# tvlearn/evo

Hardware: AMD Instinct MI355X
Metric: E-step candidate-state evals/sec (NxS), full EM iteration (higher is better)
Workload: dtype f64; 1 GPU; ES3C D=256 H=512 S=200 N=100k f64 (north-star shape); algo=es3c, N_total=100000, N_rank0=100000, D=256, H=512, S=200, step=10 full EM iterations, world_size_rccl=1, ea=fit/randflip 10 parents x 1 child x 1 gen, states=p_init_Kn=1/H (init_states default), rng=device, mstep=device, parallelism=dp1

## Files before the change

evo_amd/csrc/evo_amd.hip:

```cpp
#include "../../include/evo_amd.h"

#include <dlfcn.h>
#include <math.h>
#include <stdarg.h>
#include <stdio.h>
#include <stdlib.h>
#include <string.h>

#include <chrono>
#include <memory>
#include <string>
#include <vector>

#include "common.hpp"
#include "gemm_f64.hpp"
#include "kernels_bsc.hpp"
#include "kernels_common.hpp"
#include "kernels_evolve.hpp"
#include "kernels_mstep.hpp"
#include "kernels_sssc.hpp"
#include "kernels_sssc_quad.hpp"
#include "kernels_fused.hpp"

static thread_local char g_err[512] = "";
// ... 110 lines not shown
  bool gemm_forked = false;
  hipStream_t stream_copy = nullptr;
  hipEvent_t ev_theta = nullptr, ev_theta_done = nullptr;
  hipEvent_t ev_mbox = nullptr, ev_bak = nullptr;
  int mbox_side = 1;
  int theta_copy_engine = 0;
  double rel_frac = -1.0;
  bool ar_gemm_pending = false;
  int overlap_gemm = 1;
  int early_fork = -1;
  int bg_unit = 0;
  int fold_clear = 1;
  bool acc_clean = false, clist_clean = false;
  bool wq_copy_valid = false;
  double *gram_diag_out = nullptr;
  bool gram_diag_written = false;
  bool mbox_fold_req = false;
  unsigned long long mbox_folded_seq = 0;
  int stats_chunks = 1;
  int n_cu = 256;
  int stats_stage = 1;
  int stats_waves = 0;
  PairBins pbins = {};
  int bins_min = 256;
 int bins_scale = 3;
  int bins_scale_cur = 0;
  int bins_auto = 1;
  int bins_nwg = 2048;
  int bsc_wave_opt = 1;
  int gemm_ws_opt = 1;
  double *gemm_ws = nullptr;
  size_t gemm_ws_n = 0;
  int pair_bins = 1;
  int gemm_streamk = 1;
  int fork_spare = 0;
  int sk_spare = -1;
  int sssc_prec32 = 0;
  int main_unstaged = 1;
  int sing_screen = 1;
  double *huge = nullptr;
  int *huge_ctl = nullptr;
  int huge_slots = 0, huge_kc = 0;
  int *sing_gen = nullptr;
  int theta_gen = 0;
  int gemm_grouped = 1;
  int gemm_per_xcd = 0;
  double grid_scale = 1.0;
  double *census = nullptr;
  i64 pre_n = 4;
  hipEvent_t ev_chunk[16] = {};
  bool configured = false, have_data = false, have_params = false, have_cand = false, B_valid = false;
  bool need_known = false;
  bool res_need[3] = {true, true, true};
  double res_cnt[3] = {0, 0, 0};
  bool cand_from_device = false;
  bool lists_clean = false;
  int pending_skip = 0;
  bool conservative_levels = false;
  int pays_agreed = -1;
  int k8_mode = -1;
  bool bsc_direct = false;
  bool f32_opt = false, f32 = false;
  float *Yf = nullptr, *Ytf = nullptr, *Wf = nullptr, *Bf = nullptr, *Esf = nullptr;
  i64 ldYt = 0;
  double *Yt = nullptr;
  int b_tn_opt = 1;
// ... 221 lines not shown
  HIP_TRY(hipEventCreateWithFlags(&c->ev_theta, hipEventDisableTiming));
  HIP_TRY(hipEventCreateWithFlags(&c->ev_theta_done, hipEventDisableTiming));
  HIP_TRY(hipEventCreateWithFlags(&c->ev_mbox, hipEventDisableTiming));
  HIP_TRY(hipEventCreateWithFlags(&c->ev_bak, hipEventDisableTiming));
  for (int i = 0; i < 16; i++) HIP_TRY(hipEventCreateWithFlags(&c->ev_chunk[i], hipEventDisableTiming));

  HIP_TRY(hipFuncSetAttribute((const void *)sssc_stats_flat_kernel, hipFuncAttributeMaxDynamicSharedMemorySize, 150 * 1024));
  HIP_TRY(hipFuncSetAttribute((const void *)sssc_big_kernel<0>, hipFuncAttributeMaxDynamicSharedMemorySize,
                              136 * 1024));
  HIP_TRY(hipFuncSetAttribute((const void *)sssc_big_kernel<0, 0>, hipFuncAttributeMaxDynamicSharedMemorySize,
                              136 * 1024));
  HIP_TRY(hipFuncSetAttribute((const void *)sssc_big_kernel<0, 1>, hipFuncAttributeMaxDynamicSharedMemorySize,
                              136 * 1024));
  HIP_TRY(hipFuncSetAttribute((const void *)sssc_big_kernel<1>, hipFuncAttributeMaxDynamicSharedMemorySize,
                              136 * 1024));
  HIP_TRY(hipFuncSetAttribute((const void *)gemm_tn128_f64, hipFuncAttributeMaxDynamicSharedMemorySize,
                              (int)GEMM128_LDS_BYTES));
  HIP_TRY(hipFuncSetAttribute((const void *)gemm_tn128_rows_f64, hipFuncAttributeMaxDynamicSharedMemorySize,
                              (int)GEMM128_LDS_BYTES));
  HIP_TRY(hipFuncSetAttribute((const void *)gemm_tn128_sk_f64, hipFuncAttributeMaxDynamicSharedMemorySize,
                              (int)GEMM128_LDS_BYTES));
  HIP_TRY(hipFuncSetAttribute((const void *)gemm_tn128_sk_f32, hipFuncAttributeMaxDynamicSharedMemorySize,
                              (int)GEMM128_LDS_BYTES));
  HIP_TRY(hipFuncSetAttribute((const void *)gemm_tn128_store_f32, hipFuncAttributeMaxDynamicSharedMemorySize,
                              (int)GEMM128_LDS_BYTES));
  {
    const void *wk[] = {(const void *)sssc_stats_wave_kernel<0, 4>,  (const void *)sssc_stats_wave_kernel<1, 4>,
                        (const void *)sssc_stats_wave_kernel<2, 4>,  (const void *)sssc_stats_wave_kernel<4, 4>,
                        (const void *)sssc_stats_wave_kernel<8, 4>,  (const void *)sssc_stats_wave_kernel<16, 4>,
                        (const void *)sssc_stats_wave_kernel<0, 1>,  (const void *)sssc_stats_wave_kernel<0, 8>,
                        (const void *)sssc_stats_wave_kernel<0, 16>};
    for (const void *f : wk) HIP_TRY(hipFuncSetAttribute(f, hipFuncAttributeMaxDynamicSharedMemorySize, 150 * 1024));
    HIP_TRY(hipFuncSetAttribute((const void *)pair_bins_reduce_kernel, hipFuncAttributeMaxDynamicSharedMemorySize, 3 * PB_TILE * 8));
    HIP_TRY(hipFuncSetAttribute((const void *)sssc_small_kernel<4, 1, 2, 256>, hipFuncAttributeMaxDynamicSharedMemorySize, 120 * 1024));
    HIP_TRY(hipFuncSetAttribute((const void *)sssc_small_kernel<8, 1, 2, 256>, hipFuncAttributeMaxDynamicSharedMemorySize, 120 * 1024));
  }
  {
    const void *fk[] = {(const void *)sssc_estep_fused_kernel<1, false>,  (const void *)sssc_estep_fused_kernel<1, true>,
                        (const void *)sssc_estep_fused_kernel<2, false>,  (const void *)sssc_estep_fused_kernel<2, true>,
                        (const void *)sssc_estep_fused_kernel<4, false>,  (const void *)sssc_estep_fused_kernel<4, true>,
                        (const void *)sssc_estep_fused_kernel<8, false>,  (const void *)sssc_estep_fused_kernel<8, true>,
                        (const void *)sssc_estep_fused_kernel<16, false>, (const void *)sssc_estep_fused_kernel<16, true>};
    for (const void *fp : fk) HIP_TRY(hipFuncSetAttribute(fp, hipFuncAttributeMaxDynamicSharedMemorySize, 160 * 1024));
  }
  *out = c;
  return 0;
}

static void free_all(evoamd_ctx *c) {
  void *ptrs[] = {c->Y,      c->yy,     c->y2sum,   c->states,  c->cand,     c->lpj,       c->cand_lpj,
                  c->cand_counts, c->flags, c->rowmax, c->rowsum, c->partial, c->partial2, c->diag, c->stage,    c->W,
                  c->Wt,     c->G,      c->Psi,     c->Bm,      c->mus,      c->pilbar_v,  c->GP,      c->DG,    c->D1,    c->PT,   c->yhat,  c->tmpWt,  c->mask_infr,  c->mask_x,  c->Yrec,
                  c->pies,   c->tmpA,    c->tmpB,    c->tmpC,    c->gjwork,  c->colpart,
                  c->acc_base, c->Es,     c->list1,   c->list2,    c->list3,    c->list_n,    c->err,
                  c->tmp_y,  c->tmp_lpj, c->tmp_states, c->dig, c->cand_dig, c->lpj_alt, c->cand_raw, c->dupold, c->gen_start,
                  c->pbins.ent, c->pbins.part, c->pbins.gcnt, c->gemm_ws, c->Yt, c->Yf, c->Ytf, c->Wf, c->Bf, c->Esf,
                  c->clist, c->clist_n, c->ovf_rec, c->theta_bak, c->rowF, c->rowcnt, c->defer, c->fpart, c->huge, c->huge_ctl};
  for (void *p : ptrs)
    if (p) (void)hipFree(p);
  if (c->h_acc) (void)hipHostFree(c->h_acc);
  if (c->h_par) (void)hipHostFree(c->h_par);
  if (c->h_theta) (void)hipHostFree(c->h_theta);
  c->h_theta = nullptr;
  if (c->h_err) (void)hipHostFree(c->h_err);
  if (c->h_dpar) (void)hipHostFree(c->h_dpar);
}

extern "C" void evoamd_ctx_destroy(evoamd_ctx *c) {
  if (!c) return;
  (void)hipSetDevice(c->device);
  (void)hipStreamSynchronize(c->stream);
  if (c->comm && g_rccl.CommDestroy) g_rccl.CommDestroy(c->comm);
  for (auto &s : c->spans) {
    (void)hipEventDestroy(s.a);
    (void)hipEventDestroy(s.b);
  }
  for (auto e : c->pool) (void)hipEventDestroy(e);
  free_all(c);
  (void)hipStreamDestroy(c->stream);
  if (c->stream2) (void)hipStreamDestroy(c->stream2);
  if (c->stream_copy) (void)hipStreamDestroy(c->stream_copy);
  if (c->ev_theta) (void)hipEventDestroy(c->ev_theta);
  if (c->ev_theta_done) (void)hipEventDestroy(c->ev_theta_done);
  if (c->ev_mbox) (void)hipEventDestroy(c->ev_mbox);
  if (c->ev_bak) (void)hipEventDestroy(c->ev_bak);
  if (c->ev_fork) (void)hipEventDestroy(c->ev_fork);
  if (c->ev_join) (void)hipEventDestroy(c->ev_join);
  for (int i = 0; i < 16; i++)
    if (c->ev_chunk[i]) (void)hipEventDestroy(c->ev_chunk[i]);
// ... 14 lines not shown
  }
  if (strcmp(name, "bsc_direct") == 0) {
    c->bsc_direct = value != 0;
    c->have_params = false;
    return 0;
  }
  if (strcmp(name, "reconstruct_in_stats") == 0) {
    c->rec_in_stats = value != 0;
    return 0;
  }
  if (strcmp(name, "prefetch_lpj") == 0) {
    c->prefetch_lpj = value != 0;
    return 0;
  }
  if (strcmp(name, "inverse_block") == 0) {
    if (value != 0 && value != 16 && value != 32) return fail(EVOAMD_E_INVALID, "inverse_block: 0 (auto), 16 or 32");
    c->spd_block = value;
    return 0;
  }
  if (strcmp(name, "overlap_gemm") == 0) {
    c->overlap_gemm = value;
    return 0;
  }
  if (strcmp(name, "stats_stage") == 0) {
    c->stats_stage = value;
    return 0;
  }
  if (strcmp(name, "stats_waves") == 0) {
    c->stats_waves = value;
    return 0;
  }
  if (strcmp(name, "pair_bins") == 0) {
    c->pair_bins = value;
    return 0;
  }
  if (strcmp(name, "gemm_streamk") == 0) {
    c->gemm_streamk = value;
    return 0;
  }
  if (strcmp(name, "b_transposed") == 0) {
    c->b_tn_opt = value;
    return 0;
  }
  if (strcmp(name, "pair_bins_scale") == 0) {
    if (value < 1 || value > 64) return fail(EVOAMD_E_INVALID, "pair_bins_scale: 1 .. 64");
    c->bins_scale = value;
    return 0;
  }
  if (strcmp(name, "pair_bins_nwg") == 0) {
    if (value < 256 || value > 2048 || (value % 256) != 0) return fail(EVOAMD_E_INVALID, "pair_bins_nwg: 256 .. 2048, multiple of 256");
    c->bins_nwg = value;
    return 0;
  }
  if (strcmp(name, "pair_bins_auto") == 0) {
    c->bins_auto = value != 0;
    return 0;
  }
  if (strcmp(name, "pair_bins_min") == 0) {
    c->bins_min = value;
    return 0;
  }
  if (strcmp(name, "bsc_stats_wave") == 0) {
    c->bsc_wave_opt = value;
    return 0;
  }
  if (strcmp(name, "gemm_workspace") == 0) {
// ... 99 lines not shown
  return (c->model == EVOAMD_MODEL_BSC) ? H * D + H * H + H + 1 + 8 : 2 * H + 4 * H * H + D * H + D + 8;
}
struct AccLayout {
  i64 Wp, Wq, pies, sigma;
  i64 xs, xss, xsz, xszsz, s_sz, sz_sz, sWp, y2;
  i64 tail;
};
static AccLayout acc_layout(const evoamd_ctx *c) {
  AccLayout a = {};
  const i64 H = c->H, D = c->D;
  if (c->model == EVOAMD_MODEL_BSC) {
    a.Wp = 0;
    a.Wq = H * D;
    a.pies = a.Wq + H * H;
    a.sigma = a.pies + H;
    a.tail = a.sigma + 1;
  } else {
    a.xs = 0;
    a.xss = H;
    a.xsz = a.xss + H * H;
    a.xszsz = a.xsz + H;
    a.sWp = a.xszsz + H * H;
    a.s_sz = a.sWp + D * H;
    a.sz_sz = a.s_sz + H * H;
    a.y2 = a.sz_sz + H * H;
    a.tail = a.y2 + D;
  }
  return a;
}

static int alloc_pair_bins(evoamd_ctx *c, int scale) {
  const i64 N = c->N;
  const int H = c->H, S = c->S;
  if (c->pbins.ent) (void)hipFree(c->pbins.ent);
  if (c->pbins.gcnt) (void)hipFree(c->pbins.gcnt);
  if (c->pbins.part) (void)hipFree(c->pbins.part);
  c->pbins = PairBins{};
  c->bins_scale_cur = 0;
  if (H >= 2 && H <= 1024) {
    PairBins pb = {};
    pb.rf = std::max(1, PB_TILE / (2 * H));
    const int nfold = (H - 1 + 1) / 2;
    pb.nb = (int)cdiv(nfold, pb.rf);
    pb.nwg = c->bins_nwg;
    pb.nsh = std::max((i64)N * S >= (i64)8 << 20 ? 8 : 4, std::min(PB_NSH_MAX, 256 / std::max(1, pb.nb)));
    pb.cap = (int)std::max<i64>(64, (i64)scale * cdiv((i64)N * S, (i64)pb.nb * pb.nwg));
    const size_t ne = (size_t)pb.nb * pb.nwg * pb.cap;
    const bool got = hipMalloc((void **)&pb.ent, ne * sizeof(double4)) == hipSuccess &&
                     hipMalloc((void **)&pb.part, (size_t)pb.nb * pb.nsh * 3 * 2 * pb.rf * H * sizeof(double)) == hipSuccess &&
                     hipMalloc((void **)&pb.gcnt, (size_t)pb.nb * pb.nwg * sizeof(int)) == hipSuccess;
    if (got) {
      HIP_TRY(hipMemsetAsync(pb.gcnt, 0, (size_t)pb.nb * pb.nwg * sizeof(int), c->stream));
      c->pbins = pb;
      c->bins_scale_cur = scale;
    } else {
      (void)hipGetLastError();
      if (pb.ent) (void)hipFree(pb.ent);
      if (pb.part) (void)hipFree(pb.part);
      if (pb.gcnt) (void)hipFree(pb.gcnt);
    }
  }
  return 0;
}

static int ensure_bins_capacity(evoamd_ctx *c) {
  if (c->model != EVOAMD_MODEL_SSSC || !c->need_known || !c->pbins.ent || c->bins_auto == 0) return 0;
  const double NS = (double)c->N * c->S;
  const double n34 = c->res_cnt[0] - c->res_cnt[1], n58 = c->res_cnt[1] - c->res_cnt[2];
  const double entries = (NS - c->res_cnt[0]) + 6.0 * n34 + 28.0 * n58;
  int want = (int)std::ceil(3.0 * 1.25 * entries / NS);
  if (want > 64) want = 64;
  if (want <= c->bins_scale_cur) return 0;
  HIP_TRY(hipStreamSynchronize(c->stream));
  if (c->stream2) HIP_TRY(hipStreamSynchronize(c->stream2));
  const int before = c->bins_scale_cur;
  int r = alloc_pair_bins(c, want);
  if (r) return r;
  if (!c->pbins.ent) {
    r = alloc_pair_bins(c, before);
    if (r) return r;
    c->bins_auto = 0;
  }
  return 0;
}

extern "C" int evoamd_configure(evoamd_ctx *c, int model, int64_t N, int D, int H, int S, int S_perm,
                                int Cmax) {
  REQUIRE(c, "ctx is NULL");
  REQUIRE(model == EVOAMD_MODEL_BSC || model == EVOAMD_MODEL_SSSC, "unknown model");
  REQUIRE(N > 0 && D > 0 && H > 0 && S > 0, "N, D, H, S must be positive");
  REQUIRE(S_perm == 0 || S_perm == 1, "S_perm must be 0 or 1");
  REQUIRE(Cmax >= 1 && Cmax <= 64 * VK_MAX_C_PER_LANE, "Cmax must be in [1, 256]");
// ... 1775 lines not shown
  bool need[3] = {true, true, true};
  int cap = 0;
  if (c->model == EVOAMD_MODEL_SSSC) {
    Batch b = {c->states, nullptr, c->Y, c->Bm, c->yy, N, c->S, 0, nullptr, c->L, c->S_perm, c->flags, KID_STATS, 0};
    b.mask = c->mask_infr;
    sa = sssc_args(c, b);
    sa.lpj_in = c->lpj;
    sa.rowmax = c->rowmax;
    sa.rowsum = c->rowsum;
    sa.Es = Es;
    sa.Ez = Ez;
    sa.Ed = Ed;
    sa.ldE = c->ldY;
    sa.xss = c->acc + a.xss;
    sa.xszsz = c->acc + a.xszsz;
    sa.xss_o = c->acc_base + c->pre_n;
    sa.xszsz_o = c->acc_base + c->pre_n + (size_t)H * H;
    if (!masked) sa.cs = c->acc_base + 4;
    cap = (int)list_cap(N * (i64)c->S);
    levels_for(c, 1, need);
    r = zero_lists(c);
    if (r) return r;
  }
  const ListOut o1 = {c->list1, c->list_n + 0 * LIST_SHARDS, cap}, o2 = {c->list2, c->list_n + 1 * LIST_SHARDS, cap},
                o3 = {c->list3, c->list_n + 2 * LIST_SHARDS, cap};
  const ListIn i1 = {o1.items, o1.counts, cap}, i2 = {o2.items, o2.counts, cap}, i3 = {o3.items, o3.counts, cap};
  const ListOut none_out = {nullptr, nullptr, 0};
  const double *Ywp = c->Y;
  int ldwp = c->ldY;
  PairBins pb = {};
  if (c->model == EVOAMD_MODEL_SSSC && !masked && c->pbins.ent &&
      (c->pair_bins == 2 || (c->pair_bins == 1 && N * (i64)c->S >= (i64)c->bins_min * 1024)))
    pb = c->pbins;

  bool bsc_wave = false;
  int bsc_grid = 0;
  PairBins bsc_pb = {};
  for (int ci = 0; ci < nchunks; ci++) {
    const i64 n0 = (i64)ci * rows_per_chunk;
    const i64 nc = std::min<i64>(rows_per_chunk, N - n0);
    const int blk0 = (int)(n0 / rpb), nblk_c = (int)cdiv(nc, rpb);
    c->grid_scale = (double)nc / (double)N;
    if (c->model == EVOAMD_MODEL_BSC) {
      const u64 *bdig = dig_for(c, c->states);
      const int SRb = (int)cdiv(c->S, 64);
      bsc_wave = c->bsc_wave_opt && bdig && (SRb == 1 || SRb == 2 || SRb == 4 || SRb == 3) && nchunks == 1 &&
                 (size_t)5 * H * sizeof(double) <= 150 * 1024;
      if (bsc_wave) {
        SpanGuard g(c, KID_STATS);
        const size_t ldsb = (size_t)5 * H * sizeof(double);
        int per_cu = (int)((160 * 1024) / (ldsb + 2048));
        if (per_cu > 8) per_cu = 8;
        if (per_cu < 1) per_cu = 1;
        bsc_pb = PairBins{};
        if (c->pbins.ent && (c->pair_bins == 2 || (c->pair_bins == 1 && N * (i64)c->S >= (i64)c->bins_min * 1024))) bsc_pb = c->pbins;
        int sgrid = (int)std::min<i64>(cdiv(nc, 4), (i64)c->n_cu * per_cu * 2);
        if (sgrid > 2048) sgrid = 2048;
        if (bsc_pb.ent && sgrid > bsc_pb.nwg) sgrid = bsc_pb.nwg;
        bsc_grid = sgrid;
        void *EsP = c->f32 ? (void *)c->Esf : (void *)c->Es;
        double *csb = c->acc_base + 4;
#define BSC_WAVE(SR)                                                                                                      \
  bsc_stats_wave_kernel<SR><<<sgrid, 256, ldsb, c->stream>>>(c->states, c->lpj, c->rowmax, c->rowsum, c->yy, nc, c->S,     \
                                                            c->S_perm, H, c->HW, c->dpar, EsP, c->acc + a.Wq, c->partial2, \
                                                            bdig, c->f32 ? 1 : 0, bsc_pb, csb)
        if (SRb == 1) BSC_WAVE(1);
// ... 74 lines not shown
      sc.states = sa.states + (size_t)n0 * c->S * c->HW;
      if (sa.dig) sc.dig = sa.dig + (size_t)n0 * c->S;
      sc.Bm = sa.Bm + (size_t)n0 * H;
      sc.yy = sa.yy + n0;
      sc.lpj_in = sa.lpj_in + (size_t)n0 * sa.ldo;
      sc.rowmax = sa.rowmax + n0;
      sc.rowsum = sa.rowsum + n0;
      sc.Es = sa.Es + (size_t)n0 * sa.ldE;
      sc.Ez = sa.Ez + (size_t)n0 * sa.ldE;
      sc.Ed = sa.Ed + (size_t)n0 * sa.ldE;
      sc.N = nc;
      const i64 total = nc * (i64)c->S;
      if (ci > 0) {
        census_lists_kernel<<<1, 256, 0, c->stream>>>(c->list_n, LIST_SHARDS, skip_mask(need), c->err, c->census);
        HIP_TRY(hipGetLastError());
      }
      const int ccap = (int)list_cap(total);
      const ListIn cA = {c->clist, c->clist_n, ccap}, cB = {c->clist + c->clist_words, c->clist_n + LIST_SHARDS, ccap},
                   cC = {c->clist + 2 * c->clist_words, c->clist_n + 2 * LIST_SHARDS, ccap};
      int flatG = 0;
      size_t flat_lds = 0;
      if (census && c->stats_flat && c->S <= FLAT_T && (H % 2) == 0 && (D % 2) == 0 && sc.Ez == sc.Es + H && c->stats_waves == 0) {
        flatG = FLAT_T / c->S;
        const int gmax = (int)(((size_t)140 * 1024 / sizeof(double) - (size_t)7 * H) / ((size_t)4 * H + 4));
        if (flatG > gmax) flatG = gmax;
        if (flatG > 4 * FLAT_T / H) flatG = 4 * FLAT_T / H;
        if (flatG >= 1) flat_lds = ((size_t)H * (4 * flatG + 7) + 4 * flatG) * sizeof(double);
      }
      const bool few4 = census && flatG < 1 && few_above4(c, c->cand_from_device ? 1 : 2);
      if (flatG >= 1 && pb.ent) {
        const i64 per_bin = (i64)pb.nwg * pb.cap;
        pb.nwg = std::min(pb.nwg, c->n_cu);
        pb.cap = (int)std::min<i64>(per_bin / pb.nwg, 1 << 30);
      }
      if (census) {
        r = ensure_census(c);
        if (r) return r;
        if (need[0] || need[1]) {
          SpanGuard g(c, KID_STATS_OVF);
          const int tg = c->cand_from_device ? 1 : 2;
          const unsigned gcap = pb.ent ? (unsigned)std::min(2048, pb.nwg) : 2048u;
          const size_t dl = (size_t)H * sizeof(double);
          if (need[0]) {
            SpanGuard gl(c, KID_STATS_K34);
            sssc_quad_kernel<1, 1, 2><<<quad_grid(c, 0, tg, total, gcap), 256, dl, c->stream>>>(sc, cA, none_out, o3, pb, c->ovf_rec);
          }
          if (need[1] && !few4) {
            SpanGuard gl(c, KID_STATS_K58);
            sssc_quad_kernel<2, 1, 2><<<quad_grid(c, 1, tg, total, gcap), 256, dl, c->stream>>>(sc, cB, none_out, o3, pb, c->ovf_rec);
          }
          HIP_TRY(hipGetLastError());
          DBG_SYNC(c, "sssc stats quad levels");
        }
      }
      if (flatG >= 1) {
        SpanGuard g(c, KID_STATS);
        int fgrid = (int)std::min<i64>(cdiv(nc, flatG), (i64)c->n_cu);
        if (pb.ent && fgrid > pb.nwg) fgrid = pb.nwg;
        sssc_stats_flat_kernel<<<fgrid, FLAT_T, flat_lds, c->stream>>>(sc, pb, c->ovf_rec, flatG);
        HIP_TRY(hipGetLastError());
        DBG_SYNC(c, "sssc stats main (flat)");
      } else {
        int Wv = (size_t)(4 * 2 + 3) * H * sizeof(double) <= 150 * 1024 ? 4 : 1;
        if (c->stats_waves == 4 || c->stats_waves == 8 || c->stats_waves == 16) Wv = c->stats_waves;
        size_t lds = (size_t)(Wv * 2 + 3) * H * sizeof(double);
        const size_t lds_static = 1024 + (size_t)Wv * 512 + 128;
// ... 63 lines not shown
        }
      } else if (need[0] || need[1] || need[2]) {
        SpanGuard g(c, KID_STATS_OVF);
        const int tg = c->cand_from_device ? 1 : 2;
        const size_t cs_lds = sc.cs ? (size_t)3 * H * sizeof(double) : 0;
        bool merged23 = false;
        if (need[0])
          sssc_small_kernel<4, 1, 2, 256><<<level_grid(c, 0, tg, total, 1024, 256), 256, cs_lds, c->stream>>>(sc, i1, o2, pb, o3);
        if (c->k8_mode == 1) {
          if (need[1])
            sssc_small_kernel<8, 1, 2, 256><<<level_grid(c, 1, tg, total, 256, 256), 256, cs_lds, c->stream>>>(sc, i2, o3, pb, o3);
        } else if (need[1] && few_dense_states(c, tg)) {
          sssc_big_kernel<1><<<level_grid(c, 1, tg, total * 256, 1024, 1), 64, big_lds(SSSC_KCAP), c->stream>>>(
              sc, i2, none_out, SSSC_KCAP, i3);
          served3 = true;
          merged23 = true;
        } else if (need[1]) {
          sssc_big_kernel<1><<<level_grid(c, 1, tg, total * 256, 4096, 1), 64, big_lds(8), c->stream>>>(sc, i2, o3, 8);
        }
        if ((need[2] || c->sing_screen) && !merged23) {
          sssc_big_kernel<1><<<level_grid(c, 2, tg, total * 256, 1024, 1), 64, big_lds(SSSC_KCAP), c->stream>>>(
              sc, i3, none_out, SSSC_KCAP);
          served3 = true;
        }
        HIP_TRY(hipGetLastError());
        DBG_SYNC(c, "sssc stats overflow levels");
      }
      if (second_stream && nchunks == 1 && early && !masked) {
        HIP_TRY(hipEventRecord(c->ev_chunk[0], main_stream));
        early_recorded = true;
      }
      if (pb.ent) {
        SpanGuard g(c, KID_STATS);
        pair_bins_reduce_kernel<<<pb.nb * pb.nsh, PB_RTHREADS, (size_t)3 * 2 * pb.rf * H * sizeof(double), c->stream>>>(pb, H, ci > 0);
        HIP_TRY(hipGetLastError());
        DBG_SYNC(c, "pair bins reduce");
      }
      skipped = skip_mask(need) & ~(served3 ? 4 : 0);
    }
    c->grid_scale = 1.0;
    if (ci == nchunks - 1) {
      {
        SpanGuard g(c, KID_MISC);
        if (c->model == EVOAMD_MODEL_BSC) {
          TailArgs ta = {};
          if (nchunks == 1 && !masked && !c->reduce_pending) {
            ta = make_tail_args(c, a, N, false, skipped);
            tail_done = true;
          }
          double *wq_copy = (!c->comm && !masked && c->tmpA) ? c->tmpA : nullptr;
          c->wq_copy_valid = wq_copy != nullptr;
          const unsigned fgrid = cdiv((i64)H * H, 256) + (tail_done ? 1 : 0);
          if (bsc_wave)
            bsc_finish_kernel<<<fgrid, 256, 0, c->stream>>>(c->acc + a.Wq, c->acc + a.pies, c->acc_base + 4, BSC_CS_SLICES, H,
                                                             c->partial2, bsc_grid, c->acc + a.sigma, bsc_pb, ta, wq_copy);
          else
            bsc_finish_kernel<<<fgrid, 256, 0, c->stream>>>(c->acc + a.Wq, c->acc + a.pies, c->colpart, nblk, H, c->partial2,
                                                             cdiv(N, 4), c->acc + a.sigma, PairBins{}, ta, wq_copy);
        } else {
          const i64 nthr = (i64)H * H > D ? (i64)H * H : D;
          TailArgs ta = {};
          if (nchunks == 1 && !masked && !c->reduce_pending) {
            ta = make_tail_args(c, a, N, census, skipped);
            tail_done = true;
          }
          sssc_finish_kernel<<<cdiv(nthr, 256) + (tail_done ? 1 : 0), 256, 0, c->stream>>>(
              c->acc + a.xss, c->acc + a.xszsz, c->acc + a.xs, c->acc + a.xsz, masked ? c->colpart : sa.cs,
// ... 785 lines not shown
```

evo_amd/csrc/kernels_sssc.hpp:

```cpp
#pragma once
#include "common.hpp"
#include "kernels_mstep.hpp"
#include "pair_bins.hpp"

struct __attribute__((aligned(64))) PairEntry {
  double g01;
  double L;
  double l00, l01, l10, l11;
  double pad[2];
};
__device__ __forceinline__ bool pair_singular_L(double L) { return L == __builtin_inf(); }
__device__ __forceinline__ bool pair_singular_lam(double l00) { return !(fabs(l00) <= 1.7976931348623157e308); }

struct __attribute__((aligned(16))) OvfRec {
  unsigned short idx[8];
  double qn;
  double pad;
  double z[8];
};
static_assert(sizeof(OvfRec) == 96, "OvfRec is six 16-byte loads");

#define CS_SLICES 16
struct SsscArgs {
  const u64 *states;
// ... 730 lines not shown
  for (int p = 0; p < PPT; p++) {
    if (live[p] && !over[p]) {
      const int k = ktot[p];
      const double *Bn = STAGEB ? Bs + (size_t)nloc[p] * a.H
                                : a.Bm + (n_first + nloc[p]) * (i64)a.H;
      const double val = sssc_k2_value(k, idx0[p], idx1[p], D1t, Bn, pe[p], yyn[p], s, a.err);
      unsigned fl = 0;
      const i64 n = n_first + nloc[p];
      a.lpj_out[n * a.ldo + a.col0 + c[p]] = clamp_lpj(val, fl);
      if (fl) {
        atomicOr(&a.flags[n], fl);
        atomicOr(&a.err[1], 1);
      }
    }
  }
  if (APPEND) append_end<BS>(lo, shard, ovf_buf, ovf_ctl, a.err);
}

template <int HWT, int W, bool CEN = false>
__global__ __launch_bounds__(64 * W, W == 4 ? 2 : 1) void sssc_stats_wave_kernel(SsscArgs a, ListOut lo, PairBins pb, int stage,
                                                                                const OvfRec *__restrict__ rec = nullptr,
                                                                                const int rec_kmax = 8) {
  a.s2inv = a.dpar[DP_S2INV];
  extern __shared__ double wrows[];
  __shared__ int bcnt[PB_MAX_BINS];
  constexpr int OVB = 64;
  __shared__ int obuf[W][2 * OVB];
  const int H = a.H, lane = lane_id(), wave = wave_id_uniform();
  double *rowS = wrows + (size_t)wave * 2 * H, *rowZ = rowS + H;
  double *accS = wrows + (size_t)W * 2 * H, *accZ = accS + H, *accD = accZ + H;
  double *rowB = accD + H + (size_t)wave * H;
  double4 *d1s = (double4 *)(accD + H + (size_t)W * H);
  const bool binned = pb.ent != nullptr;
  for (int i = threadIdx.x; i < 3 * H; i += 64 * W) accS[i] = 0.0;
  if (HWT > 0 || stage)
    for (int i = threadIdx.x; i < H; i += 64 * W) d1s[i] = a.D1[i];
  if (binned)
    for (int i = threadIdx.x; i < pb.nb; i += 64 * W) bcnt[i] = CEN ? pb.gcnt[(size_t)i * pb.nwg + blockIdx.x] : 0;
  __syncthreads();
  const int shard = (int)(blockIdx.x & (LIST_SHARDS - 1));
  const double s = a.s2inv;
  int ocnt = 0;
  auto flush_obuf = [&]() {
    int base = 0;
    if (lane == 0) base = atomicAdd(&lo.counts[shard], ocnt);
    base = __shfl(base, 0, 64);
    for (int i = lane; i < ocnt; i += 64) {
      const int pos = base + i;
      if (pos >= 0 && pos < lo.cap)
        lo.items[(i64)shard * lo.cap + pos] = obuf[wave][i];
      else
        atomicOr(a.err, EVO_ERR_LIST_FULL);
    }
    ocnt = 0;
    lds_wave_fence();
  };
  constexpr bool PF = HWT > 0;
  constexpr int HB = PF ? HWT : 1;
  struct Pre {
    double rmax, rsum, B[HB], l[4];
    u64 d[4];
  };
  auto issue = [&](i64 nn, Pre &p) {
    p.rmax = a.rowmax[nn];
    p.rsum = a.rowsum[nn];
    const double *Bnn = a.Bm + nn * H;
#pragma unroll
    for (int i = 0; i < HB; i++) {
      const int h = lane + 64 * i;
      p.B[i] = Bnn[h < H ? h : H - 1];
    }
// ... 128 lines not shown
          const double qn = q / rsum;
          const double4 d0 = D1t[idx0[u]];
          const double b0 = Bn[idx0[u]];
          double g01 = 0.0, l00 = d0.w, l01 = 0.0, l10 = 0.0, l11 = 0.0, mu1 = 0.0, g11 = 0.0, bb1 = 0.0;
          if (pair[u]) {
            const double4 d1 = D1t[idx1[u]];
            g01 = pe[u].g01;
            l00 = pe[u].l00;
            l01 = pe[u].l01;
            l10 = pe[u].l10;
            l11 = pe[u].l11;
            mu1 = d1.x;
            g11 = d1.z;
            bb1 = Bn[idx1[u]];
            if (pair_singular_lam(pe[u].l00)) atomicOr(a.err, 2);
          }
          const double mu0 = d0.x;
          const double v0 = b0 - d0.z * mu0 - g01 * mu1;
          const double v1 = bb1 - g01 * mu0 - g11 * mu1;
          const double k0 = s * (l00 * v0 + l01 * v1) + mu0;
          const double k1 = s * (l10 * v0 + l11 * v1) + mu1;
          unsafeAtomicAdd(&rowS[idx0[u]], qn);
          unsafeAtomicAdd(&rowZ[idx0[u]], qn * k0);
          unsafeAtomicAdd(&accD[idx0[u]], qn * (l00 + k0 * k0));
          if (pair[u]) {
            unsafeAtomicAdd(&rowS[idx1[u]], qn);
            unsafeAtomicAdd(&rowZ[idx1[u]], qn * k1);
            unsafeAtomicAdd(&accD[idx1[u]], qn * (l11 + k1 * k1));
            const double pq = qn, pv = qn * (l01 + k0 * k1);
            const i64 o01 = (i64)idx0[u] * H + idx1[u];
            if (!binned) {
              unsafeAtomicAdd(&a.xss[o01], pq);
              unsafeAtomicAdd(&a.xszsz[o01], pv);
            } else {
              const double pw = qn * (l10 + k1 * k0);
              if (!pb_append(pb, bcnt, blockIdx.x, H, idx0[u], idx1[u], pq, pv, pw)) {
                unsafeAtomicAdd(&a.xss_o[o01], pq);
                unsafeAtomicAdd(&a.xszsz_o[o01], pv);
                unsafeAtomicAdd(&a.xszsz_o[(i64)idx1[u] * H + idx0[u]], pw);
              }
            }
          }
        }
      }
      if (CEN) {
        auto add_rec = [&](const OvfRec &r, int kk) {
          if (r.qn != 0.0) {
#pragma unroll
            for (int i = 0; i < 8; i++)
              if (i < kk) {
                const int h = (int)r.idx[i];
                unsafeAtomicAdd(&rowS[h], r.qn);
                unsafeAtomicAdd(&rowZ[h], r.z[i]);
              }
          }
        };
        if (ofirst >= 0) {
          int kk = 0;
#pragma unroll
          for (int u = 0; u < RG; u++) kk = (u == ofirst) ? k[u] : kk;
          add_rec(orec, kk);
        }
        if (__ballot(omore) != 0ull) {
#pragma unroll
          for (int u = 1; u < RG; u++)
            if (over[u] && k[u] <= rec_kmax && u != ofirst) {
// ... 6 lines not shown
#pragma unroll
        for (int u = 0; u < RG; u++)
          if (over[u]) {
            const int e = (int)(n * a.C + c0 + 64 * u + lane);
            if (o_direct) {
              const int pos = obase + my_off[u];
              if (pos >= 0 && pos < lo.cap)
                lo.items[(i64)shard * lo.cap + pos] = e;
              else
                atomicOr(a.err, EVO_ERR_LIST_FULL);
            } else {
              obuf[wave][ocnt + my_off[u]] = e;
            }
          }
        if (!o_direct) {
          ocnt += n_over;
          if (ocnt >= OVB) {
            lds_wave_fence();
            flush_obuf();
          }
        }
      }
    };
    if (PF) {
      group(0, std::true_type{});
      for (int c0 = 4 * 64; c0 < a.C; c0 += 4 * 64) group(c0, std::false_type{});
    } else {
      for (int c0 = 0; c0 < a.C; c0 += 4 * 64) group(c0, std::false_type{});
    }
    lds_wave_fence();
    double *es = a.Es + n * a.ldE, *ez = a.Ez + n * a.ldE;
    for (int h = lane; h < H; h += 64) {
      const double vs = rowS[h], vz = rowZ[h];
      es[h] = vs;
      ez[h] = vz;
      if (vs != 0.0) {
        unsafeAtomicAdd(&accS[h], vs);
        unsafeAtomicAdd(&accZ[h], vz);
      }
    }
    lds_wave_fence();
  }
  if (ocnt) flush_obuf();
  __syncthreads();
  double *sl = a.cs + (size_t)(blockIdx.x % CS_SLICES) * 3 * H;
  for (int h = threadIdx.x; h < H; h += 64 * W) {
    if (accS[h] != 0.0) {
      unsafeAtomicAdd(&sl[h], accS[h]);
      unsafeAtomicAdd(&sl[H + h], accZ[h]);
    }
    if (accD[h] != 0.0) unsafeAtomicAdd(&sl[2 * H + h], accD[h]);
  }
  if (binned)
    for (int i = threadIdx.x; i < pb.nb; i += 64 * W) {
      const int cnt = bcnt[i];
      pb.gcnt[(size_t)i * pb.nwg + blockIdx.x] = cnt < pb.cap ? cnt : pb.cap;
    }
}

__global__ __launch_bounds__(256) void finish_sym_kernel(double *__restrict__ xss,
                                                              const double *__restrict__ xs, int H) {
  const i64 t = (i64)blockIdx.x * 256 + threadIdx.x;
  if (t >= (i64)H * H) return;
  const int i = (int)(t / H), j = (int)(t - (i64)i * H);
  if (i == j)
    xss[t] = xs[i];
  else if (i > j)
    xss[t] = xss[(i64)j * H + i];
}

template <int BAR>
__device__ __forceinline__ void big_bar() {
  if (BAR == 2)
    __syncthreads();
  else if (BAR == 1)
    lds_barrier();
  else
    lds_wave_fence();
}
template <int BAR, class F>
__device__ __forceinline__ void rows_of(const int lane, const int k, F f) {
  if (BAR == 2) {
    for (int r = lane; r < k; r += 64) f(r);
  } else {
    if (lane < k) f(lane);
  }
}
template <int BAR>
__device__ __forceinline__ int wave_idamax(const double *M, const int k, const int p, const int lane, double &m) {
// ... 536 lines not shown
                                                          const double *__restrict__ part, int nblk, int H,
                                                          const double *__restrict__ y2sum, double *__restrict__ y2out,
                                                          int D, const double *__restrict__ xss_o,
                                                          const double *__restrict__ xszsz_o,
                                                          const PairEntry *__restrict__ PT, PairBins pb,
                                                          TailArgs ta = TailArgs{}) {
  if (ta.tail && blockIdx.x == gridDim.x - 1) {
    tail_body(ta);
    return;
  }
  const i64 t = (i64)blockIdx.x * 256 + threadIdx.x;
  if (t < D) y2out[t] = y2sum[t];
  if (t >= (i64)H * H) return;
  const int i = (int)(t / H), j = (int)(t - (i64)i * H);
  const bool wide = H >= 3;
  if (i == j) {
    const double s = ordered_strided_sum(part + i, 3 * (i64)H, nblk);
    xs[i] = s;
    xss[t] = s;
  }
  if (wide ? (j == (i + 1 == H ? 0 : i + 1)) : (i == j)) xsz[i] = ordered_strided_sum(part + H + i, 3 * (i64)H, nblk);
  if (wide ? (j == (i + 2 >= H ? i + 2 - H : i + 2)) : (i == j))
    xszsz[(i64)i * H + i] = ordered_strided_sum(part + 2 * H + i, 3 * (i64)H, nblk);
  if (i < j) {
    const i64 tl = (i64)j * H + i;
    const double uss = xss[t], u = xszsz[t];
    double lower = u;
    if (PT && uss != 0.0) {
      const PairEntry pe = PT[t];
      lower = u + (pe.l10 - pe.l01) * uss;
    }
    double bq = 0.0, bu = 0.0, bl = 0.0;
    if (pb.part) pb_collect(pb, H, i, j, bq, bu, bl);
    const double ss = uss + xss_o[t] + bq;
    xss[t] = ss;
    xss[tl] = ss;
    xszsz[t] = u + xszsz_o[t] + bu;
    xszsz[tl] = lower + xszsz_o[tl] + bl;
  }
}

__global__ __launch_bounds__(256) void set_diag_kernel(double *__restrict__ M, const double *__restrict__ d, int H) {
  const int h = blockIdx.x * 256 + threadIdx.x;
  if (h < H) M[(i64)h * H + h] = d[h];
}

__global__ __launch_bounds__(256) void sssc_tables_kernel(const double *__restrict__ G, const double *__restrict__ Psi,
                                                          const double *__restrict__ mus,
                                                          const double *__restrict__ pil_bar,
                                                          const double *__restrict__ dpar, int H,
                                                          double4 *__restrict__ D1, PairEntry *__restrict__ PT,
                                                          double2 *__restrict__ GP, double4 *__restrict__ DG,
                                                          int *__restrict__ sing_gen, int gen) {
  const i64 t = (i64)blockIdx.x * 256 + threadIdx.x;
  if (t >= (i64)H * H) return;
  const int h0 = (int)(t / H), h1 = (int)(t - (i64)h0 * H);
  const double s = dpar[DP_S2INV];
  GP[t] = make_double2(G[t], Psi[t]);
  if (h0 == h1) {
    const double g = G[t], p = Psi[t];
    DG[h0] = make_double4(mus[h0], pil_bar[h0], g, p);
    const double T = 1.0 + s * p * g;
    double4 d = make_double4(mus[h0], pil_bar[h0] - 0.5 * log(fabs(T)), g, p / T);
    if (p == 0.0) {
      d.y = __builtin_inf();
      d.w = (s * g != 0.0) ? 1.0 / (s * g) : 0.0;
// ... 39 lines not shown
```

evo_amd/csrc/pair_bins.hpp:

```cpp
#pragma once
#include "common.hpp"

#define PB_TILE 4096
#define PB_MAX_BINS 256
#define PB_NSH_MAX 16
#define PB_RTHREADS 1024
struct PairBins {
  double4 *ent;
  int *gcnt;
  double *part;
  int cap, nb, rf, nwg;
  int nsh;
};
__device__ __forceinline__ int pb_fold(int i, int H) { return i < H - 2 - i ? i : H - 2 - i; }

__device__ __forceinline__ bool pb_append(const PairBins &pb, int *bcnt, int wg, int H, int i, int j, double q,
                                          double vu, double vl) {
  const int f = pb_fold(i, H);
  const int bin = f / pb.rf;
  const int pos = atomicAdd(&bcnt[bin], 1);
  if (pos >= pb.cap) return false;
  const int r = 2 * (f - bin * pb.rf) + (i != f ? 1 : 0);
  const size_t at = ((size_t)bin * pb.nwg + wg) * pb.cap + pos;
  pb.ent[at] = make_double4(q, vu, vl, __longlong_as_double((long long)(((unsigned)r << 16) | (unsigned)j)));
  return true;
}

__global__ __launch_bounds__(PB_RTHREADS) void pair_bins_reduce_kernel(PairBins pb, int H, int accumulate) {
  extern __shared__ double pb_tile[];
  constexpr int NW = PB_RTHREADS / 64;
  __shared__ int pre_sh[NW][65];
  const int NSH = pb.nsh;
  const int bin = blockIdx.x / NSH, sh = blockIdx.x - bin * NSH;
  const int slots = 2 * pb.rf * H;
  double *tq = pb_tile, *tu = pb_tile + slots, *tl = pb_tile + 2 * slots;
  for (int i = threadIdx.x; i < 3 * slots; i += PB_RTHREADS) pb_tile[i] = 0.0;
  lds_barrier();
  const int lane = lane_id(), wave = wave_id_uniform();
  for (int j0 = 0; sh + NSH * (wave + NW * j0) < pb.nwg; j0 += 64) {
    const int w = sh + NSH * (wave + NW * (j0 + lane));
    int n = 0;
    if (w < pb.nwg) {
      const size_t reg = (size_t)bin * pb.nwg + w;
      n = pb.gcnt[reg];
      if (n > pb.cap) n = pb.cap;
      if (n != 0) pb.gcnt[reg] = 0;
    }
    int incl = n;
#pragma unroll
    for (int o = 1; o < 64; o <<= 1) {
      const int t = __shfl_up(incl, o, 64);
      if (lane >= o) incl += t;
    }
    pre_sh[wave][lane + 1] = incl;
    if (lane == 0) pre_sh[wave][0] = 0;
    lds_wave_fence();
    const int T = pre_sh[wave][64];
// ... 4 lines not shown
      for (int u = 0; u < 4; u++) {
        const int t = t0 + 64 * u + lane;
        on[u] = t < T;
        int lo = 0, hi = 64;
#pragma unroll
        for (int it = 0; it < 6; it++) {
          const int mid = (lo + hi) >> 1;
          if (pre_sh[wave][mid] <= t)
            lo = mid;
          else
            hi = mid;
        }
        const int wr = sh + NSH * (wave + NW * (j0 + lo));
        const size_t at = on[u] ? ((size_t)bin * pb.nwg + wr) * pb.cap + (t - pre_sh[wave][lo]) : 0;
        v[u] = pb.ent[at];
      }
#pragma unroll
      for (int u = 0; u < 4; u++)
        if (on[u]) {
          const unsigned k = (unsigned)__double_as_longlong(v[u].w);
          const int t = (int)(k >> 16) * H + (int)(k & 0xFFFFu);
          unsafeAtomicAdd(&tq[t], v[u].x);
          unsafeAtomicAdd(&tu[t], v[u].y);
          unsafeAtomicAdd(&tl[t], v[u].z);
        }
    }
    lds_wave_fence();
  }
  lds_barrier();
  double *out = pb.part + (size_t)blockIdx.x * 3 * slots;
  for (int i = threadIdx.x; i < 3 * slots; i += PB_RTHREADS) out[i] = accumulate ? out[i] + pb_tile[i] : pb_tile[i];
}

__device__ __forceinline__ void pb_collect(const PairBins &pb, int H, int i, int j, double &bq, double &bu, double &bl) {
  const int f = pb_fold(i, H), bin = f / pb.rf;
  const int slots = 2 * pb.rf * H;
  const int slot = (2 * (f - bin * pb.rf) + (i != f ? 1 : 0)) * H + j;
  const double *p = pb.part + (size_t)bin * pb.nsh * 3 * slots + slot;
  bq = bu = bl = 0.0;
  for (int sh = 0; sh < pb.nsh; sh++, p += 3 * slots) {
    bq += p[0];
    bu += p[slots];
    bl += p[2 * slots];
  }
}
```

Measured before the change: 5.102 billion state evals/s.

## Add compact pair records for two-active-unit SSSC states with split reduction

Adds a second binning path for pair (two-active-unit) contributions. Each record stores (q, k) as a double2 plus a 16-bit slot key, replacing the double4 entry, and the per-pair l01/l10 terms are reconstructed at collection time from the PT table. A new reduce kernel handles the general bins in two half-tile blocks, coordinated by atomicOr on the counter, while separate blocks reduce the pair records. The Es/Ez stores become nontemporal. The aim is to cut record bandwidth and LDS footprint in the stats reduction, at the cost of more buffers, a more complex reduction and extra algebra in the collect step.

```diff
diff --git a/evo_amd/csrc/evo_amd.hip b/evo_amd/csrc/evo_amd.hip
--- a/evo_amd/csrc/evo_amd.hip
+++ b/evo_amd/csrc/evo_amd.hip
@@ -166,6 +166,8 @@
   double *gemm_ws = nullptr;
   size_t gemm_ws_n = 0;
   int pair_bins = 1;
+  int pair_records = 1;
+  int pair_pnsh = 0;
   int gemm_streamk = 1;
   int fork_spare = 0;
   int sk_spare = -1;
@@ -453,6 +455,7 @@
                         (const void *)sssc_stats_wave_kernel<0, 16>};
     for (const void *f : wk) HIP_TRY(hipFuncSetAttribute(f, hipFuncAttributeMaxDynamicSharedMemorySize, 150 * 1024));
     HIP_TRY(hipFuncSetAttribute((const void *)pair_bins_reduce_kernel, hipFuncAttributeMaxDynamicSharedMemorySize, 3 * PB_TILE * 8));
+    HIP_TRY(hipFuncSetAttribute((const void *)pair_bins_reduce2_kernel, hipFuncAttributeMaxDynamicSharedMemorySize, 2 * PB_TILE * 8));
     HIP_TRY(hipFuncSetAttribute((const void *)sssc_small_kernel<4, 1, 2, 256>, hipFuncAttributeMaxDynamicSharedMemorySize, 120 * 1024));
     HIP_TRY(hipFuncSetAttribute((const void *)sssc_small_kernel<8, 1, 2, 256>, hipFuncAttributeMaxDynamicSharedMemorySize, 120 * 1024));
   }
@@ -475,7 +478,7 @@
                   c->pies,   c->tmpA,    c->tmpB,    c->tmpC,    c->gjwork,  c->colpart,
                   c->acc_base, c->Es,     c->list1,   c->list2,    c->list3,    c->list_n,    c->err,
                   c->tmp_y,  c->tmp_lpj, c->tmp_states, c->dig, c->cand_dig, c->lpj_alt, c->cand_raw, c->dupold, c->gen_start,
-                  c->pbins.ent, c->pbins.part, c->pbins.gcnt, c->gemm_ws, c->Yt, c->Yf, c->Ytf, c->Wf, c->Bf, c->Esf,
+                  c->pbins.ent, c->pbins.part, c->pbins.gcnt, c->pbins.pent, c->pbins.pkey, c->pbins.pcnt, c->pbins.ppart, c->gemm_ws, c->Yt, c->Yf, c->Ytf, c->Wf, c->Bf, c->Esf,
                   c->clist, c->clist_n, c->ovf_rec, c->theta_bak, c->rowF, c->rowcnt, c->defer, c->fpart, c->huge, c->huge_ctl};
   for (void *p : ptrs)
     if (p) (void)hipFree(p);
@@ -556,6 +559,15 @@
   }
   if (strcmp(name, "pair_bins") == 0) {
     c->pair_bins = value;
+    return 0;
+  }
+  if (strcmp(name, "pair_records") == 0) {
+    c->pair_records = value != 0;
+    return 0;
+  }
+  if (strcmp(name, "pair_bins_pnsh") == 0) {
+    if (value < 0 || value > PB_NSH_MAX) return fail(EVOAMD_E_INVALID, "pair_bins_pnsh: 0 .. 16");
+    c->pair_pnsh = value;
     return 0;
   }
   if (strcmp(name, "gemm_streamk") == 0) {
@@ -721,32 +733,41 @@
 static int alloc_pair_bins(evoamd_ctx *c, int scale) {
   const i64 N = c->N;
   const int H = c->H, S = c->S;
-  if (c->pbins.ent) (void)hipFree(c->pbins.ent);
-  if (c->pbins.gcnt) (void)hipFree(c->pbins.gcnt);
-  if (c->pbins.part) (void)hipFree(c->pbins.part);
+  for (void *p : {(void *)c->pbins.ent, (void *)c->pbins.gcnt, (void *)c->pbins.part, (void *)c->pbins.pent,
+                  (void *)c->pbins.pkey, (void *)c->pbins.pcnt, (void *)c->pbins.ppart})
+    if (p) (void)hipFree(p);
   c->pbins = PairBins{};
   c->bins_scale_cur = 0;
   if (H >= 2 && H <= 1024) {
     PairBins pb = {};
-    pb.rf = std::max(1, PB_TILE / (2 * H));
+    pb.rf = pb_rows_per_bin(H);
     const int nfold = (H - 1 + 1) / 2;
     pb.nb = (int)cdiv(nfold, pb.rf);
     pb.nwg = c->bins_nwg;
     pb.nsh = std::max((i64)N * S >= (i64)8 << 20 ? 8 : 4, std::min(PB_NSH_MAX, 256 / std::max(1, pb.nb)));
     pb.cap = (int)std::max<i64>(64, (i64)scale * cdiv((i64)N * S, (i64)pb.nb * pb.nwg));
-    const size_t ne = (size_t)pb.nb * pb.nwg * pb.cap;
-    const bool got = hipMalloc((void **)&pb.ent, ne * sizeof(double4)) == hipSuccess &&
-                     hipMalloc((void **)&pb.part, (size_t)pb.nb * pb.nsh * 3 * 2 * pb.rf * H * sizeof(double)) == hipSuccess &&
-                     hipMalloc((void **)&pb.gcnt, (size_t)pb.nb * pb.nwg * sizeof(int)) == hipSuccess;
+    pb.pcap = (int)std::max<i64>(64, (i64)3 * cdiv((i64)N * S, (i64)pb.nb * pb.nwg));
+    pb.pnsh = c->pair_pnsh > 0 ? c->pair_pnsh : pb.nsh;
+    const size_t ne = (size_t)pb.nb * pb.nwg * pb.cap, np = (size_t)pb.nb * pb.nwg * pb.pcap;
+    const bool pair = c->model == EVOAMD_MODEL_SSSC;
+    bool got = hipMalloc((void **)&pb.ent, ne * sizeof(double4)) == hipSuccess &&
+               hipMalloc((void **)&pb.part, (size_t)pb.nb * pb.nsh * 3 * 2 * pb.rf * H * sizeof(double)) == hipSuccess &&
+               hipMalloc((void **)&pb.gcnt, (size_t)pb.nb * pb.nwg * sizeof(int)) == hipSuccess;
+    if (got && pair)
+      got = hipMalloc((void **)&pb.pent, np * sizeof(double2)) == hipSuccess &&
+            hipMalloc((void **)&pb.pkey, np * sizeof(unsigned short)) == hipSuccess &&
+            hipMalloc((void **)&pb.ppart, (size_t)pb.nb * pb.pnsh * 2 * 2 * pb.rf * H * sizeof(double)) == hipSuccess &&
+            hipMalloc((void **)&pb.pcnt, (size_t)pb.nb * pb.nwg * sizeof(int)) == hipSuccess;
     if (got) {
       HIP_TRY(hipMemsetAsync(pb.gcnt, 0, (size_t)pb.nb * pb.nwg * sizeof(int), c->stream));
+      if (pb.pcnt) HIP_TRY(hipMemsetAsync(pb.pcnt, 0, (size_t)pb.nb * pb.nwg * sizeof(int), c->stream));
       c->pbins = pb;
       c->bins_scale_cur = scale;
     } else {
       (void)hipGetLastError();
-      if (pb.ent) (void)hipFree(pb.ent);
-      if (pb.part) (void)hipFree(pb.part);
-      if (pb.gcnt) (void)hipFree(pb.gcnt);
+      for (void *p : {(void *)pb.ent, (void *)pb.part, (void *)pb.gcnt, (void *)pb.pent, (void *)pb.pkey, (void *)pb.pcnt,
+                      (void *)pb.ppart})
+        if (p) (void)hipFree(p);
     }
   }
   return 0;
@@ -2588,6 +2609,15 @@
   if (c->model == EVOAMD_MODEL_SSSC && !masked && c->pbins.ent &&
       (c->pair_bins == 2 || (c->pair_bins == 1 && N * (i64)c->S >= (i64)c->bins_min * 1024)))
     pb = c->pbins;
+  if (pb.pent && c->pair_records) {
+    if (c->need_known) {
+      const double n34 = c->res_cnt[0] - c->res_cnt[1], n58 = c->res_cnt[1] - c->res_cnt[2];
+      if (6.0 * n34 + 28.0 * n58 <= (double)N * c->S / 16.0) pb.nsh = std::min(pb.nsh, 2);
+    }
+  } else {
+    pb.pent = nullptr;
+    pb.ppart = nullptr;
+  }
 
   bool bsc_wave = false;
   int bsc_grid = 0;
@@ -2728,6 +2758,9 @@
         const i64 per_bin = (i64)pb.nwg * pb.cap;
         pb.nwg = std::min(pb.nwg, c->n_cu);
         pb.cap = (int)std::min<i64>(per_bin / pb.nwg, 1 << 30);
+        pb.nsh = c->pbins.nsh;
+        pb.pent = nullptr;
+        pb.ppart = nullptr;
       }
       if (census) {
         r = ensure_census(c);
@@ -2857,7 +2890,11 @@
       }
       if (pb.ent) {
         SpanGuard g(c, KID_STATS);
-        pair_bins_reduce_kernel<<<pb.nb * pb.nsh, PB_RTHREADS, (size_t)3 * 2 * pb.rf * H * sizeof(double), c->stream>>>(pb, H, ci > 0);
+        if (pb.pent)
+          pair_bins_reduce2_kernel<<<pb.nb * (2 * pb.nsh + pb.pnsh), PB_RTHREADS, (size_t)2 * 2 * pb.rf * H * sizeof(double),
+                                     c->stream>>>(pb, H, ci > 0);
+        else
+          pair_bins_reduce_kernel<<<pb.nb * pb.nsh, PB_RTHREADS, (size_t)3 * 2 * pb.rf * H * sizeof(double), c->stream>>>(pb, H, ci > 0);
         HIP_TRY(hipGetLastError());
         DBG_SYNC(c, "pair bins reduce");
       }
diff --git a/evo_amd/csrc/kernels_sssc.hpp b/evo_amd/csrc/kernels_sssc.hpp
--- a/evo_amd/csrc/kernels_sssc.hpp
+++ b/evo_amd/csrc/kernels_sssc.hpp
@@ -786,11 +786,12 @@
   double *rowB = accD + H + (size_t)wave * H;
   double4 *d1s = (double4 *)(accD + H + (size_t)W * H);
   const bool binned = pb.ent != nullptr;
+  const bool precs = binned && pb.pent != nullptr;
   for (int i = threadIdx.x; i < 3 * H; i += 64 * W) accS[i] = 0.0;
   if (HWT > 0 || stage)
     for (int i = threadIdx.x; i < H; i += 64 * W) d1s[i] = a.D1[i];
   if (binned)
-    for (int i = threadIdx.x; i < pb.nb; i += 64 * W) bcnt[i] = CEN ? pb.gcnt[(size_t)i * pb.nwg + blockIdx.x] : 0;
+    for (int i = threadIdx.x; i < pb.nb; i += 64 * W) bcnt[i] = CEN && !precs ? pb.gcnt[(size_t)i * pb.nwg + blockIdx.x] : 0;
   __syncthreads();
   const int shard = (int)(blockIdx.x & (LIST_SHARDS - 1));
   const double s = a.s2inv;
@@ -985,6 +986,12 @@
             if (!binned) {
               unsafeAtomicAdd(&a.xss[o01], pq);
               unsafeAtomicAdd(&a.xszsz[o01], pv);
+            } else if (precs) {
+              if (!pb_append_pair(pb, bcnt, blockIdx.x, H, idx0[u], idx1[u], pq, qn * (k0 * k1))) {
+                unsafeAtomicAdd(&a.xss_o[o01], pq);
+                unsafeAtomicAdd(&a.xszsz_o[o01], pv);
+                unsafeAtomicAdd(&a.xszsz_o[(i64)idx1[u] * H + idx0[u]], qn * (l10 + k1 * k0));
+              }
             } else {
               const double pw = qn * (l10 + k1 * k0);
               if (!pb_append(pb, bcnt, blockIdx.x, H, idx0[u], idx1[u], pq, pv, pw)) {
@@ -1057,8 +1064,8 @@
     double *es = a.Es + n * a.ldE, *ez = a.Ez + n * a.ldE;
     for (int h = lane; h < H; h += 64) {
       const double vs = rowS[h], vz = rowZ[h];
-      es[h] = vs;
-      ez[h] = vz;
+      __builtin_nontemporal_store(vs, &es[h]);
+      __builtin_nontemporal_store(vz, &ez[h]);
       if (vs != 0.0) {
         unsafeAtomicAdd(&accS[h], vs);
         unsafeAtomicAdd(&accZ[h], vz);
@@ -1079,7 +1086,10 @@
   if (binned)
     for (int i = threadIdx.x; i < pb.nb; i += 64 * W) {
       const int cnt = bcnt[i];
-      pb.gcnt[(size_t)i * pb.nwg + blockIdx.x] = cnt < pb.cap ? cnt : pb.cap;
+      if (precs)
+        pb.pcnt[(size_t)i * pb.nwg + blockIdx.x] = cnt < pb.pcap ? cnt : pb.pcap;
+      else
+        pb.gcnt[(size_t)i * pb.nwg + blockIdx.x] = cnt < pb.cap ? cnt : pb.cap;
     }
 }
 
@@ -1682,6 +1692,16 @@
     }
     double bq = 0.0, bu = 0.0, bl = 0.0;
     if (pb.part) pb_collect(pb, H, i, j, bq, bu, bl);
+    if (pb.ppart) {
+      double pq, pk;
+      pb_collect_pairs(pb, H, i, j, pq, pk);
+      if (pq != 0.0) {
+        const PairEntry pe = PT[t];
+        bq += pq;
+        bu += pk + pe.l01 * pq;
+        bl += pk + pe.l10 * pq;
+      }
+    }
     const double ss = uss + xss_o[t] + bq;
     xss[t] = ss;
     xss[tl] = ss;
diff --git a/evo_amd/csrc/pair_bins.hpp b/evo_amd/csrc/pair_bins.hpp
--- a/evo_amd/csrc/pair_bins.hpp
+++ b/evo_amd/csrc/pair_bins.hpp
@@ -11,18 +11,42 @@
   double *part;
   int cap, nb, rf, nwg;
   int nsh;
+  double2 *pent;
+  unsigned short *pkey;
+  int *pcnt;
+  double *ppart;
+  int pcap, pnsh;
 };
-__device__ __forceinline__ int pb_fold(int i, int H) { return i < H - 2 - i ? i : H - 2 - i; }
+__host__ __device__ __forceinline__ int pb_rows_per_bin(int H) { return PB_TILE / (2 * H) > 1 ? PB_TILE / (2 * H) : 1; }
+__host__ __device__ __forceinline__ int pb_fold(int i, int H) { return i < H - 2 - i ? i : H - 2 - i; }
+__host__ __device__ __forceinline__ int pb_place(int i, int j, int H, int rf, int &slot) {
+  const int f = pb_fold(i, H);
+  const int bin = f / rf;
+  slot = (2 * (f - bin * rf) + (i != f ? 1 : 0)) * H + j;
+  return bin;
+}
 
 __device__ __forceinline__ bool pb_append(const PairBins &pb, int *bcnt, int wg, int H, int i, int j, double q,
                                           double vu, double vl) {
-  const int f = pb_fold(i, H);
-  const int bin = f / pb.rf;
+  int slot;
+  const int bin = pb_place(i, j, H, pb.rf, slot);
   const int pos = atomicAdd(&bcnt[bin], 1);
   if (pos >= pb.cap) return false;
-  const int r = 2 * (f - bin * pb.rf) + (i != f ? 1 : 0);
+  const int r = slot / H;
   const size_t at = ((size_t)bin * pb.nwg + wg) * pb.cap + pos;
   pb.ent[at] = make_double4(q, vu, vl, __longlong_as_double((long long)(((unsigned)r << 16) | (unsigned)j)));
+  return true;
+}
+
+__device__ __forceinline__ bool pb_append_pair(const PairBins &pb, int *bcnt, int wg, int H, int i, int j, double q,
+                                               double kk) {
+  int slot;
+  const int bin = pb_place(i, j, H, pb.rf, slot);
+  const int pos = atomicAdd(&bcnt[bin], 1);
+  if (pos >= pb.pcap) return false;
+  const size_t at = ((size_t)bin * pb.nwg + wg) * pb.pcap + pos;
+  pb.pent[at] = make_double2(q, kk);
+  pb.pkey[at] = (unsigned short)slot;
   return true;
 }
 
@@ -93,6 +117,136 @@
   for (int i = threadIdx.x; i < 3 * slots; i += PB_RTHREADS) out[i] = accumulate ? out[i] + pb_tile[i] : pb_tile[i];
 }
 
+template <int U, typename Take, typename Load, typename Add>
+__device__ __forceinline__ void pb_walk(int nwg, int cap, int bin, int sh, int nsh, int nw, int *pre, Take take, Load load,
+                                        Add add) {
+  const int lane = lane_id(), wave = wave_id_uniform();
+  using V = decltype(load((size_t)0));
+  for (int j0 = 0; sh + nsh * (wave + nw * j0) < nwg; j0 += 64) {
+    const int w = sh + nsh * (wave + nw * (j0 + lane));
+    int n = 0;
+    if (w < nwg) {
+      n = take((size_t)bin * nwg + w);
+      if (n > cap) n = cap;
+    }
+    int incl = n;
+#pragma unroll
+    for (int o = 1; o < 64; o <<= 1) {
+      const int t = __shfl_up(incl, o, 64);
+      if (lane >= o) incl += t;
+    }
+    pre[lane + 1] = incl;
+    if (lane == 0) pre[0] = 0;
+    lds_wave_fence();
+    const int T = pre[64];
+    for (int t0 = 0; t0 < T; t0 += 64 * U) {
+      V v[U];
+      bool on[U];
+#pragma unroll
+      for (int u = 0; u < U; u++) {
+        const int t = t0 + 64 * u + lane;
+        on[u] = t < T;
+        int lo = 0, hi = 64;
+#pragma unroll
+        for (int it = 0; it < 6; it++) {
+          const int mid = (lo + hi) >> 1;
+          if (pre[mid] <= t)
+            lo = mid;
+          else
+            hi = mid;
+        }
+        const int wr = sh + nsh * (wave + nw * (j0 + lo));
+        const size_t at = on[u] ? ((size_t)bin * nwg + wr) * cap + (t - pre[lo]) : 0;
+        v[u] = load(at);
+      }
+#pragma unroll
+      for (int u = 0; u < U; u++)
+        if (on[u]) add(v[u]);
+    }
+    lds_wave_fence();
+  }
+}
+
+__global__ __launch_bounds__(PB_RTHREADS, 8) void pair_bins_reduce2_kernel(PairBins pb, int H, int accumulate) {
+  extern __shared__ double pb_tile[];
+  constexpr int NW = PB_RTHREADS / 64;
+  __shared__ int pre_sh[NW][65];
+  const int slots = 2 * pb.rf * H;
+  const int wave = wave_id_uniform();
+  const int ngen = 2 * pb.nb * pb.nsh;
+  if ((int)blockIdx.x < ngen) {
+    const int bin = blockIdx.x / (2 * pb.nsh), rem = blockIdx.x - bin * 2 * pb.nsh;
+    const int sh = rem >> 1, h = rem & 1;
+    const int half = slots / 2, lo = h * half;
+    double *tq = pb_tile, *tu = pb_tile + half, *tl = pb_tile + 2 * half;
+    for (int i = threadIdx.x; i < 3 * half; i += PB_RTHREADS) pb_tile[i] = 0.0;
+    lds_barrier();
+    const unsigned mine = 1u << (30 + h), other = 1u << (31 - h);
+    pb_walk<4>(
+        pb.nwg, pb.cap, bin, sh, pb.nsh, NW, pre_sh[wave],
+        [&](size_t reg) {
+          unsigned *cp = (unsigned *)pb.gcnt + reg;
+          const unsigned old = atomicOr(cp, mine);
+          if (old & other) *cp = 0u;
+          return (int)(old & 0x3FFFFFFFu);
+        },
+        [&](size_t at) { return pb.ent[at]; },
+        [&](const double4 &v) {
+          const unsigned k = (unsigned)__double_as_longlong(v.w);
+          const int t = (int)(k >> 16) * H + (int)(k & 0xFFFFu) - lo;
+          if ((unsigned)t < (unsigned)half) {
+            unsafeAtomicAdd(&tq[t], v.x);
+            unsafeAtomicAdd(&tu[t], v.y);
+            unsafeAtomicAdd(&tl[t], v.z);
+          }
+        });
+    lds_barrier();
+    double *out = pb.part + ((size_t)bin * pb.nsh + sh) * 3 * slots + lo;
+    for (int i = threadIdx.x; i < 3 * half; i += PB_RTHREADS) {
+      const int p = i / half;
+      double *o = out + (size_t)p * slots + (i - p * half);
+      *o = accumulate ? *o + pb_tile[i] : pb_tile[i];
+    }
+    return;
+  }
+  const int b = blockIdx.x - ngen;
+  const int bin = b / pb.pnsh, sh = b - bin * pb.pnsh;
+  double *tq = pb_tile, *tk = pb_tile + slots;
+  for (int i = threadIdx.x; i < 2 * slots; i += PB_RTHREADS) pb_tile[i] = 0.0;
+  lds_barrier();
+  struct Rec {
+    double2 v;
+    unsigned k;
+  };
+  pb_walk<4>(
+      pb.nwg, pb.pcap, bin, sh, pb.pnsh, NW, pre_sh[wave],
+      [&](size_t reg) {
+        const int n = pb.pcnt[reg];
+        if (n != 0) pb.pcnt[reg] = 0;
+        return n;
+      },
+      [&](size_t at) { return Rec{pb.pent[at], (unsigned)pb.pkey[at]}; },
+      [&](const Rec &r) {
+        unsafeAtomicAdd(&tq[r.k], r.v.x);
+        unsafeAtomicAdd(&tk[r.k], r.v.y);
+      });
+  lds_barrier();
+  double *out = pb.ppart + (size_t)b * 2 * slots;
+  for (int i = threadIdx.x; i < 2 * slots; i += PB_RTHREADS) out[i] = accumulate ? out[i] + pb_tile[i] : pb_tile[i];
+}
+
+__device__ __forceinline__ void pb_collect_pairs(const PairBins &pb, int H, int i, int j, double &pq, double &pk) {
+  int slot;
+  const int bin = pb_place(i, j, H, pb.rf, slot);
+  const int slots = 2 * pb.rf * H;
+  const double *p = pb.ppart + (size_t)bin * pb.pnsh * 2 * slots + slot;
+  pq = pk = 0.0;
+  for (int sh = 0; sh < pb.pnsh; sh++, p += 2 * slots) {
+    pq += p[0];
+    pk += p[slots];
+  }
+}
+
 __device__ __forceinline__ void pb_collect(const PairBins &pb, int H, int i, int j, double &bq, double &bu, double &bl) {
   const int f = pb_fold(i, H), bin = f / pb.rf;
   const int slots = 2 * pb.rf * H;
```

Result: faster. 5.163 billion state evals/s, median of 6 (+1.2%).
